# neale/safelife-k2

Hardware: AMD Instinct MI355X
Metric: env-steps/sec (whole node) on 64×64 boards, batch 65536; bit-exact vs CPU ref (higher is better)
Workload: dtype u16; 1 GPU; 64x64 proc-gen prune-still, PPO wrapper chain; envs_per_gpu=65536, burnin_steps=400, global_batch=65536, parallelism=dp1 (env shards), obs=none, rng=philox, board_mode=auto, read_board=False

## Files before the change

include/safelife_hip.h:

```cpp
#ifndef SAFELIFE_HIP_H
#define SAFELIFE_HIP_H

#include <stdint.h>

#ifdef __cplusplus
extern "C" {
#endif

#define SL_OK 0
#define SL_EINVAL (-1)
#define SL_EHIP (-2)
#define SL_ETOOBIG (-3)

#define SL_RNG_STREAM 0
#define SL_RNG_PHILOX 1

#define SL_KERNEL_AUTO 0
#define SL_KERNEL_GENERIC 1
#define SL_KERNEL_FAST 2
#define SL_KERNEL_BANDS 3
#define SL_KERNEL_MID 4

#define SL_FAMILY_GENERIC 0
#define SL_FAMILY_SMALL_SEG4 1
// ... 139 lines not shown
    int32_t *possible;
    int32_t *side_effect;
    float *spawn_prob;
    double *min_performance;
    int32_t *prior_x;
    int32_t *prior_y;
    int32_t *prior_len;
    int32_t *prior_head;
    int32_t *exit_count;
    int16_t *exit_y, *exit_x;
    int32_t *level_index;
    int32_t *episodes;
    int32_t *num_steps;
    int32_t *spawn_flags;
    int32_t *start_roll;
    uint32_t *planes;
    int32_t *planes_ok;
    uint32_t *elig_planes;
    uint32_t *board_planes;
    uint32_t board_zero;
    int32_t planes_live;
    uint32_t agent_planes;
    uint32_t goals_gray;
} sl_env_state;

enum sl_planes_ok_bits {
    SL_POK_GOALS_MIRROR = 2,
    SL_POK_GOALS_FIXED = 4,
    SL_POK_ELIG = 8,
    SL_POK_GOALS_SIX = 16,
    SL_POK_GOALS_LEVEL = 32,
    SL_POK_BOARD_PLANES = 64,
    SL_POK_BOARD_FULL = 128,
    SL_POK_BOARD_LO12 = 256,
    SL_POK_GOALS = SL_POK_GOALS_MIRROR | SL_POK_GOALS_FIXED | SL_POK_GOALS_SIX |
                   SL_POK_GOALS_LEVEL,
    SL_POK_BOARD = SL_POK_BOARD_PLANES | SL_POK_BOARD_FULL | SL_POK_BOARD_LO12
};

typedef struct sl_level_pool {
    int32_t K, H, W;
    const uint16_t *board;
    const uint16_t *goals;
    const int32_t *agent_x, *agent_y, *orientation;
    const float *spawn_prob;
    const double *min_performance;
// ... 74 lines not shown
#define SL_PLAN_K64_BITS64 1
#define SL_PLAN_K64_PLANES 2
#define SL_PLAN_K64_GRAY 3
#define SL_PLAN_K64_W6 4
#define SL_PLAN_K64_S6 5
#define SL_PLAN_K64_CHAN 6
#define SL_PLAN_KEEP_RUNTIME 0
#define SL_PLAN_KEEP_C3 1
#define SL_PLAN_KEEP_ALL 2

typedef struct sl_step_plan {
    int32_t empty;
    int32_t family;
    int32_t replay;
    int32_t stream_phase;
    int32_t plane_mode;
    int32_t demote_first;
    int32_t obs;
    int32_t resets;
    int32_t capture;
    int32_t kernel64;
    int32_t keep;
    int32_t view_kind;
} sl_step_plan;

int sl_env_step_plan(const sl_env_state *st, const sl_level_pool *pool, const sl_env_cfg *cfg,
                     const uint8_t *info_flags, sl_step_plan *out);

int sl_env_board_sync(sl_env_state *st, void *stream);

int sl_env_reset(sl_env_state *st, const sl_level_pool *pool, const uint8_t *mask,
                 const sl_env_cfg *cfg, void *stream);

int sl_env_obs(const sl_env_state *st, int vh, int vw, int remove_white_goals,
               int obs_mode, const int32_t *channels, int nch, void *out,
               void *stream);

int sl_env_action(sl_env_state *st, const int32_t *actions, int can_toggle_powers,
                  int can_toggle_colors, int64_t *act, void *stream);
int sl_env_advance(sl_env_state *st, const sl_env_cfg *cfg, void *stream);
int sl_env_rescore(sl_env_state *st, int32_t *points, void *stream);
int sl_env_exit_colors(sl_env_state *st, int mode, void *stream);


int sl_sample_actions(const void *probs, int probs_f64, int64_t B, int A, int64_t ld,
                      int rng_mode, const double *uniforms, uint64_t seed, uint32_t env0,
// ... 12 lines not shown
```

safelife-k2_amd/csrc/sl_bits.hip:

```cpp
#include "sl_bits_geo.h"
#include "sl_env_step.h"

using namespace sl;
using namespace sl::fast;
using namespace sl::bits;

namespace {

constexpr int kMinWaves = 4;
constexpr int kMinWavesObs = 3;

constexpr int N = 64;

typedef __attribute__((address_space(3))) u32 lds_u32;

__device__ __forceinline__ void dma_board(const uint16_t *__restrict__ src, lds_u32 *buf,
                                          int lane) {
    const char *s = reinterpret_cast<const char *>(src);
#pragma unroll
    for (int k = 0; k < 8; k++) {
        const int q = k * 64 + lane, row = q >> 3, pos = q & 7;
        const int c = (pos - ((row >> 5) << 2)) & 7;
        __builtin_amdgcn_global_load_lds((const void *)(s + row * 128 + c * 16),
                                         (__attribute__((address_space(3))) void *)(buf + k * 256),
// ... 631 lines not shown
    }
    if (fx.fuse_reset && reset && lane == 0) queue_reset(fx.scratch, st.B, a.step, b);
}

template <int OBS, int MODE>
__global__ void __launch_bounds__(64, (OBS || MODE == SPAWN_STREAM) ? kMinWavesObs : kMinWaves)
k_env_step_bits64(StepKArgs ka) {
    const int64_t b = blockIdx.x;
    const int lane = threadIdx.x;
    __shared__ __attribute__((aligned(16))) u32 stage[N * N / 2];
    __shared__ __attribute__((aligned(16))) uint16_t vmask[OBS >= 2 ? sl::obs::kFusedChanCells : 2];
    __shared__ uint8_t rowlist[OBS ? 64 : 1];
    lds_u32 *buf = (lds_u32 *)&stage[0];
    Pre pre;
    issue_pre(ka.st, ka.actions, b, lane, pre);
    dma_board(ka.st.board + b * (int64_t)(N * N), buf, lane);
    step_env<OBS, MODE>(ka.st, ka.a, ka.fx, b, lane, buf, vmask, rowlist, ka.actions, ka.ctp, ka.ctc,
                        ka.reward_out, ka.done_out, ka.flags_out, ka.ep_len_out, ka.ep_rew_out,
                        pre);
}


constexpr u32 kKeepAll = 0xFFFFu, kKeepC3 = 0x877Fu, kAgentC3 = 0x0062u;
template <u32 K16>
struct PlaneSlots {
    static constexpr bool kFixed = K16 == kKeepC3;
    u32 keep;
    u32 store;
    __device__ __forceinline__ u32 keep32() const { return K16 ? K16 * 0x10001u : keep; }
    __device__ __forceinline__ u32 store32() const {
        return kFixed ? (K16 & ~kAgentC3) * 0x10001u : store;
    }
    __device__ __forceinline__ bool kept(int q) const { return (keep32() >> q) & 1u; }
    __device__ __forceinline__ bool stored(int q) const { return (store32() >> q) & 1u; }
    __device__ __forceinline__ u32 agent16() const {
        return kFixed ? kAgentC3 : (keep32() & ~store32()) & 0xFFFFu;
    }
    __device__ __forceinline__ int pos(int q) const {
        if (kFixed) return __builtin_popcount(store32() & ((1u << q) - 1u));
        u32 k = store;
        asm volatile("" : "+s"(k));
        return __builtin_popcount(k & ((1u << q) - 1u));
    }
    __device__ __forceinline__ int stored16() const { return __builtin_popcount(store32() & 0xFFFFu); }
    static __device__ __forceinline__ PlaneSlots of(u32 zero, u32 agent) {
        const u32 k = ~zero & 0xFFFFu;
        return PlaneSlots{k * 0x10001u, (k & ~agent) * 0x10001u};
    }
};
__device__ __forceinline__ void agent_words(int ay, int ax, int lane, u32 aw[2]) {
    const u32 bit = lane == 2 * (ax >> 1) + (ay >> 5) ? 1u << (ay & 31) : 0u;
    aw[0] = (ax & 1) ? 0u : bit;
    aw[1] = (ax & 1) ? bit : 0u;
}
constexpr int kMinWavesPlanes = 5;
constexpr int planes_min_waves(u32 k16, int obs) {
    return (obs == 0 && k16 == kKeepC3) ? kMinWavesPlanes : kMinWaves;
}

template <u32 K16>
__device__ __forceinline__ void dma_planes(const u32 *__restrict__ bp, PlaneSlots<K16> ps,
                                           lds_u32 *buf, int lane) {
    const int groups = (2 * ps.stored16() + 3) >> 2;
    const char *s = reinterpret_cast<const char *>(bp);
#pragma unroll
    for (int g = 0; g < 8; g++)
        if (g < groups)
            __builtin_amdgcn_global_load_lds((const void *)(s + g * 1024 + lane * 16),
                                             (__attribute__((address_space(3))) void *)(buf + g * 256),
                                             16, 0, 2);
}

__device__ __forceinline__ int near_cell_index(int k, int y0, int x0) {
    const int dy = k < 5 ? 0 : (k == 5 ? -1 : k == 6 ? 1 : k == 7 ? -2 : 2);
    const int dx = k >= 5 || k == 0 ? 0 : (k == 1 ? -1 : k == 2 ? 1 : k == 3 ? -2 : 2);
    return ((y0 + dy) & 63) * 64 + ((x0 + dx) & 63);
}
struct NearCells {
    int y0, x0;
    u32 v;
    __device__ __forceinline__ uint32_t operator()(int i) const {
        const int dy = (((i >> 6) - y0 + 32) & 63) - 32, dx = (((i & 63) - x0 + 32) & 63) - 32;
        const int k = dy == 0 ? (dx == 0 ? 0 : dx == -1 ? 1 : dx == 1 ? 2 : dx == -2 ? 3 : 4)
                              : (dy == -1 ? 5 : dy == 1 ? 6 : dy == -2 ? 7 : 8);
        return (u32)__builtin_amdgcn_readlane((int)v, __builtin_amdgcn_readfirstlane(k));
    }
};
template <u32 K16>
__device__ __forceinline__ u32 lds_plane_cell(const lds_u32 *buf, PlaneSlots<K16> ps, int i) {
    const int y = i >> 6, x = i & 63;
    const lds_u32 *q = buf + 2 * (x >> 1) + (y >> 5);
    const u32 r = (u32)(y & 31);
    const int w = 16 * (x & 1);
    u32 v = 0;
#pragma unroll
    for (int p = 0; p < 16; p++) {
        const int pw = ps.pos(p) + (w ? ps.stored16() : 0);
        if (ps.stored(p)) v |= ((q[pw * 64] >> r) & 1u) << p;
    }
    return v;
}

template <u32 K16, int OBS>
__global__ void __launch_bounds__(64, planes_min_waves(K16, OBS))
k_env_step_bits64_planes(StepKArgs ka) {
    __shared__ __attribute__((aligned(16))) u32 stage[N * N / 2];
    uint16_t *const vm = nullptr;
    constexpr bool GRAY = false, W6 = false, SPLIT_EPI = false;
#include "sl_planes64_step.inc"
}

template <u32 K16, int OBS>
__global__ void __launch_bounds__(64, planes_min_waves(K16, OBS))
k_env_planes64_gray(StepKArgs ka) {
    static_assert(OBS <= 1, "channel views load the three colour planes");
    __shared__ __attribute__((aligned(16))) u32 stage[N * N / 2];
    uint16_t *const vm = nullptr;
    constexpr bool GRAY = true, W6 = false, SPLIT_EPI = false;
#include "sl_planes64_step.inc"
}

constexpr int kMinWavesW6 = 6;
constexpr int kStageDwW6 = 1536;
template <u32 K16>
__global__ void __launch_bounds__(64, kMinWavesW6)
k_env_planes64_w6(StepKArgs ka) {
    __shared__ __attribute__((aligned(16))) u32 stage[kStageDwW6];
    uint16_t *const vm = nullptr;
    constexpr int OBS = 0;
    constexpr bool GRAY = true, W6 = true, SPLIT_EPI = false;
#include "sl_planes64_step.inc"
}

template <u32 K16>
__global__ void __launch_bounds__(64, kMinWavesW6)
k_env_planes64_s6(StepKArgs ka) {
    __shared__ __attribute__((aligned(16))) u32 stage[kStageDwW6];
    uint16_t *const vm = nullptr;
    constexpr int OBS = 0;
    constexpr bool GRAY = true, W6 = true, SPLIT_EPI = true;
#include "sl_planes64_step.inc"
}

constexpr int kTailThreads = 256;
__global__ void __launch_bounds__(kTailThreads)
k_env_epilogue_reset64(sl_env_state st, StepArgs a, sl_level_pool pool, ResetArgs ra,
                       int64_t *scratch, double *reward_out, uint8_t *done_out,
                       uint8_t *flags_out, int32_t *ep_len_out, int32_t *ep_rew_out) {
    const int64_t b = (int64_t)blockIdx.x * kTailThreads + threadIdx.x;
    const int lane = threadIdx.x & 63;
    if (b == 0) scratch[8 * st.B + 2 + ((a.step + 1) & 1)] = 0;
    bool reset = false;
    if (b < st.B) {
        const Handover h = get_handover(handover_of(scratch, st.B), b);
        const HandFields f{{st, b, a.bonus_table}, h.go, h.ax, h.ay};
        reset = epilogue_core(st, a, b, f, h.act_reward, h.points, h.score, h.possible, h.side,
                              reward_out, done_out, flags_out, ep_len_out, ep_rew_out);
    }
    __shared__ uint64_t finished[kTailThreads / 64];
    const int wave = __builtin_amdgcn_readfirstlane((int)(threadIdx.x >> 6));
    const uint64_t mine = __ballot(reset);
    if (lane == 0) finished[wave] = mine;
    __builtin_amdgcn_fence(__ATOMIC_RELEASE, "workgroup");
// ... 1 lines not shown
    const int64_t b0 = (int64_t)blockIdx.x * kTailThreads;
    int i = 0;
#pragma unroll 1
    for (int q = 0; q < kTailThreads / 64; q++) {
        const uint64_t f = finished[q];
        uint64_t todo = ((uint64_t)(u32)__builtin_amdgcn_readfirstlane((int)(f >> 32)) << 32) |
                        (u32)__builtin_amdgcn_readfirstlane((int)f);
        while (todo) {
            const int k = __builtin_ctzll(todo);
            todo &= todo - 1;
            if ((i++ & (kTailThreads / 64 - 1)) == wave) wave_reset(st, pool, ra, b0 + 64 * q + k, lane);
        }
    }
}

template <u32 K16, int ESZ>
__global__ void __launch_bounds__(64, kMinWaves)
k_env_planes64_chan(StepKArgs ka) {
    constexpr int OBS = ESZ == 1 ? 3 : (ESZ == 4 ? 4 : 2);
    __shared__ __attribute__((aligned(16))) u32 stage[N * N / 2];
    __shared__ __attribute__((aligned(16))) uint16_t vmask[sl::obs::kFusedChanCells];
    uint16_t *const vm = vmask;
    constexpr bool GRAY = false, W6 = false, SPLIT_EPI = false;
#include "sl_planes64_step.inc"
}

__global__ void __launch_bounds__(64) k_board_sync64(sl_env_state st, int demote) {
    const int64_t b = blockIdx.x;
    const int lane = threadIdx.x;
    const int pok = __builtin_amdgcn_readfirstlane(st.planes_ok[b]);
    if (!(pok & SL_POK_BOARD_PLANES)) return;
    if (!(pok & SL_POK_BOARD_FULL)) {
        const PlaneSlots<0> ps = PlaneSlots<0>::of(st.board_zero, st.agent_planes);
        const u32 *bp = st.planes + b * 4096 + lane;
        u32 P[32];
#pragma unroll
        for (int q = 0; q < 32; q++) P[q] = ps.stored(q) ? bp[ps.pos(q) * 64] : 0u;
        u32 aw[2];
        agent_words(__builtin_amdgcn_readfirstlane(st.agent_y[b]),
                    __builtin_amdgcn_readfirstlane(st.agent_x[b]), lane, aw);
#pragma unroll
        for (int q = 0; q < 32; q++)
            if ((ps.agent16() >> (q & 15)) & 1u) P[q] = aw[q >> 4];
        transpose32(P);
        u32 *gb = reinterpret_cast<u32 *>(st.board + b * (int64_t)(N * N)) + (lane & 1) * 1024 +
                  (lane >> 1);
#pragma unroll
        for (int y = 0; y < 32; y++) gb[y * 32] = P[y];
    }
    if (lane == 0)
        st.planes_ok[b] = demote ? pok & ~(SL_POK_BOARD_PLANES | SL_POK_BOARD_FULL)
                                 : pok | SL_POK_BOARD_FULL;
}

__global__ void __launch_bounds__(64)
k_stream_prologue64(StepKArgs ka) {
    const sl_env_state &st = ka.st;
    const int64_t b = blockIdx.x;
    const int lane = threadIdx.x;
    const int64_t off = b * (int64_t)(N * N);
    const int lane_off = (lane & 1) * 1024 + (lane >> 1);
    const u32 V = load_record(st, ka.actions, b, lane);
    const Scratch w = scratch_of(ka.fx.scratch, st.B);
    const int spf = rec(V, R_SPF) | (ka.ctp ? 1 : 0);
    SpawnCtx sc{0u, 0u, 0ull, 0.0};
    u32 P[32], ch[2];
// ... 93 lines not shown

void launch_planes64(int keep, int obs, unsigned grid, const StepKArgs &ka, hipStream_t s) {
    switch (keep) {
    case SL_PLAN_KEEP_C3: launch_planes64_k<kKeepC3>(obs, grid, ka, s); break;
    case SL_PLAN_KEEP_ALL: launch_planes64_k<kKeepAll>(obs, grid, ka, s); break;
    default: launch_planes64_k<0>(obs, grid, ka, s); break;
    }
}

StepKArgs kargs_of(const StepCall &c) {
    return StepKArgs{*c.st, c.a, c.fx, c.actions, c.ctp, c.ctc, c.reward, c.done, c.flags,
                     c.ep_len, c.ep_rew};
}

int counts64(const StepCall &c) {
    const sl_env_state &st = *c.st;
    const int rc = launch_env_action(st, c.actions, c.ctp, c.ctc,
                                     scratch_of(c.fx.scratch, st.B).act, c.s);
    if (rc) return rc;
    hipLaunchKernelGGL(k_stream_prologue64, dim3((unsigned)st.B), dim3(64), 0, c.s, kargs_of(c));
    return hipGetLastError() == hipSuccess ? SL_OK : SL_EHIP;
}

int step64(const StepCall &c) {
    const StepPlan &p = c.plan;
    const unsigned grid = (unsigned)c.st->B;
    const StepKArgs ka = kargs_of(c);
    hipStream_t s = c.s;
    switch (p.kernel64) {
    case SL_PLAN_K64_BITS64:
        if (p.replay) launch_bits64<SPAWN_STREAM>(p.view_kind, grid, ka, s);
        else launch_bits64<SPAWN_PHILOX>(p.view_kind, grid, ka, s);
        break;
    case SL_PLAN_K64_PLANES: launch_planes64(p.keep, p.view_kind, grid, ka, s); break;
    case SL_PLAN_K64_CHAN: launch_planes64_chan(p.keep, obs_esz(p.view_kind), grid, ka, s); break;
    case SL_PLAN_K64_GRAY:
        if (p.view_kind)
            hipLaunchKernelGGL((k_env_planes64_gray<kKeepC3, 1>), dim3(grid), dim3(64), 0, s, ka);
        else
            hipLaunchKernelGGL((k_env_planes64_gray<kKeepC3, 0>), dim3(grid), dim3(64), 0, s, ka);
        break;
    case SL_PLAN_K64_S6:
        hipLaunchKernelGGL((k_env_planes64_s6<kKeepC3>), dim3(grid), dim3(64), 0, s, ka);
        break;
    case SL_PLAN_K64_W6:
        hipLaunchKernelGGL((k_env_planes64_w6<kKeepC3>), dim3(grid), dim3(64), 0, s, ka);
        break;
    default: return SL_EINVAL;
    }
    return hipGetLastError() == hipSuccess ? SL_OK : SL_EHIP;
}
// ... 44 lines not shown
```

safelife-k2_amd/csrc/sl_env_step.hip:

```cpp
#include "sl_env_step.h"

using namespace sl;

namespace {

constexpr bool kAutoTakesMid = true;

int view_kind_of(int obs_mode) {
    switch (obs_mode) {
    case SL_OBS_PACKED: return 1;
    case SL_OBS_CHANNELS_U8: return 3;
    case SL_OBS_CHANNELS_F32: return 4;
    default: return 2;
    }
}

}

extern "C" int sl_env_step_family(int H, int W, int kernel) {
    if (H < 1 || W < 1) return SL_EINVAL;
    if (kernel != SL_KERNEL_AUTO && kernel != SL_KERNEL_GENERIC && kernel != SL_KERNEL_FAST)
        return SL_EINVAL;
    if (kernel != SL_KERNEL_GENERIC) {
        if (H == 64 && W == 64) return SL_FAMILY_BITS64;
// ... 61 lines not shown
                         p.oa.vh <= kViewMaxRows128 && p.oa.vw <= 128;
    const bool fuse64 =
        fast && cfg.obs_out &&
        ((p.oa.mode == SL_OBS_PACKED && p.oa.vh * p.oa.vw <= obs::kObsMaxCells) ||
         (p.oa.mode != SL_OBS_PACKED && p.oa.vh <= 64 && p.oa.vw <= 64 &&
          p.oa.vh * p.oa.vw + 2 <= obs::kFusedChanCells && (((uintptr_t)cfg.obs_out) & 15) == 0));
    p.obs = !cfg.obs_out ? SL_PLAN_OBS_NONE
            : fuse128    ? SL_PLAN_OBS_FUSED128
            : fuse64     ? SL_PLAN_OBS_FUSED64
                         : SL_PLAN_OBS_SEPARATE;
    const bool views_ok = p.obs != SL_PLAN_OBS_SEPARATE;
    if (fast128 && planes128)
        p.plane_mode = planes_can && views_ok && (!replay || st.elig_planes);
    else if (fast && planes64)
        p.plane_mode = planes_can && views_ok && !replay;
    p.demote_first = (planes128 || planes64) && !p.plane_mode;
    p.view_kind = (p.obs == SL_PLAN_OBS_FUSED64 || p.obs == SL_PLAN_OBS_FUSED128)
                      ? view_kind_of(p.oa.mode) : 0;

    if (fast && !p.plane_mode) {
        p.kernel64 = SL_PLAN_K64_BITS64;
    } else if (fast) {
        p.keep = planes64_keep(st);
        const bool gray = p.keep == SL_PLAN_KEEP_C3 && st.goals_gray;
        if (p.view_kind >= 2) p.kernel64 = SL_PLAN_K64_CHAN;
        else if (!gray) p.kernel64 = SL_PLAN_K64_PLANES;
        else if (p.view_kind || cfg.planes64_waves == 5) p.kernel64 = SL_PLAN_K64_GRAY;
        else if (cfg.planes64_waves != SL_PLANES64_W6_UNSPLIT && cfg.auto_reset &&
                 (reinterpret_cast<uintptr_t>(cfg.scratch) & 15) == 0)
            p.kernel64 = SL_PLAN_K64_S6;
        else p.kernel64 = SL_PLAN_K64_W6;
    }

    p.resets = !cfg.auto_reset                    ? SL_PLAN_RESETS_NONE
               : small                            ? (p.cap ? SL_PLAN_RESETS_SCAN : SL_PLAN_RESETS_IN_KERNEL)
               : p.kernel64 == SL_PLAN_K64_S6     ? SL_PLAN_RESETS_SPLIT_TAIL64
               : fast                             ? SL_PLAN_RESETS_LIST64
               : fast128                          ? SL_PLAN_RESETS_LIST128
                                                  : SL_PLAN_RESETS_SCAN;
    *out = p;
    return SL_OK;
}

extern "C" int sl_env_step_plan(const sl_env_state *st, const sl_level_pool *pool,
                                const sl_env_cfg *cfg, const uint8_t *info_flags,
                                sl_step_plan *out) {
// ... 118 lines not shown
```

safelife-k2_amd/csrc/sl_planes64_step.inc:

```
    const sl_env_state &st = ka.st;
    const StepArgs &a = ka.a;
    const FastExtra &fx = ka.fx;
    const int64_t b = blockIdx.x;
    const int lane = threadIdx.x;
    lds_u32 *buf = (lds_u32 *)&stage[0];
    const PlaneSlots<K16> ps = PlaneSlots<K16>::of(st.board_zero, st.agent_planes);
    constexpr int kStageDw = (int)(sizeof(stage) / sizeof(u32));
    static_assert(!W6 || (PlaneSlots<K16>::kFixed && OBS == 0), "W6: fixed planes, no views");
    static_assert(!W6 || 2 * __builtin_popcount(K16 & ~kAgentC3 & 0xFFFFu) * 64 <= kStageDw,
                  "the stored plane words fit the buffer");
    static_assert(pool_rows_dwords(K16 ? K16 : 0xFFFFu, W6) <= kStageDw,
                  "the pool's start-plane rows fit the buffer");
    static_assert(kStageDw >= (W6 ? N * N / 4 : N * N / 2), "a board, or half of one (W6)");
    Pre pre;
    const bool gray_blank = GRAY && (!OBS || fx.obs_rw != 0);
    if (!GRAY) issue_pre(st, ka.actions, b, lane, pre);
    else if (gray_blank) issue_pre<0>(st, ka.actions, b, lane, pre);
    else issue_pre<1>(st, ka.actions, b, lane, pre);
    dma_planes(st.planes + b * 4096, ps, buf, lane);
    const int64_t off = b * (int64_t)(N * N);
    const int lane_off = (lane & 1) * 1024 + (lane >> 1);
    u32 *gg = reinterpret_cast<u32 *>(st.goals + off) + lane_off;
    u32 *mg = st.planes + b * 4096 + 2048 + lane;
    u32 *bp = st.planes + b * 4096 + lane;
    const u32 V = pre.V;
    const int pok_all = rec(V, R_POK);
    const bool pin = (pok_all & SL_POK_BOARD_PLANES) != 0;
    u32 gcol[3][2];
#pragma unroll
    for (int k = 0; k < 3; k++) {
        gcol[k][0] = pre.g[k][0];
        gcol[k][1] = pre.g[k][1];
    }
// ... 11 lines not shown
    if (fx.pool.K > 0 && fx.pool.board_planes && st.start_roll) roll = rec(V, R_ROLL);
    wait_vm();
    if (!pin) {
        if (!W6) {
            dma_board(st.board + off, buf, lane);
            wait_vm();
        }
        u32 R[32];
        if (W6) board_pairs_halves(st.board + off, buf, lane, R);
        else read_pairs(buf, lane, R);
        transpose32(R);
#pragma unroll
        for (int q = 0; q < 32; q++)
            if (ps.stored(q)) buf[ps.pos(q) * 64 + lane] = R[q];
        __builtin_amdgcn_fence(__ATOMIC_SEQ_CST, "wavefront");
        __builtin_amdgcn_wave_barrier();
    }
    RecEnv env{st, b, rec(V, R_GO), rec(V, R_AX), rec(V, R_AY), rec(V, R_SCORE),
               rec(V, R_BASE), rec(V, R_POSS), rec_f64(V, R_MP)};
    int act_reward = 0;
    int eidx[4];
    u32 eval[4];
    const int ay0 = rec(V, R_AY), ax0 = rec(V, R_AX);
    const u32 near = lane < 9 ? lds_plane_cell(buf, ps, near_cell_index(lane, ay0, ax0)) |
                                    (lane == 0 ? ps.agent16() : 0u)
                              : 0u;
    OverlayT<NearCells> ov;
    ov.src = NearCells{ay0, ax0, near};
    ov.n = 0;
#pragma unroll
    for (int k = 0; k < 4; k++) {
        ov.idx[k] = 0;
        ov.val[k] = 0;
    }
    if (lane == 0) act_reward = act_core(env, rec(V, R_ACT), N, N, ka.ctp, ka.ctc, ov);
    int ne = ov.n;
#pragma unroll
    for (int k = 0; k < 4; k++) {
        eidx[k] = ov.idx[k];
        eval[k] = ov.val[k];
    }
    act_reward = __builtin_amdgcn_readfirstlane(act_reward);
    ne = __builtin_amdgcn_readfirstlane(ne);
#pragma unroll
    for (int k = 0; k < 4; k++) {
        eidx[k] = __builtin_amdgcn_readfirstlane(eidx[k]);
        eval[k] = (u32)__builtin_amdgcn_readfirstlane((int)eval[k]);
        if (K16) eval[k] &= K16;
        eval[k] &= ~ps.agent16();
    }
    const RecFields fl = rec_fields(a, V, __builtin_amdgcn_readfirstlane(env.go),
                                    __builtin_amdgcn_readfirstlane(env.ax),
                                    __builtin_amdgcn_readfirstlane(env.ay));

    u32 PB[32];
#pragma unroll
    for (int q = 0; q < 32; q++) PB[q] = ps.stored(q) ? buf[ps.pos(q) * 64 + lane] : 0u;
    wait_lgkm();
    constexpr u32 KEEP = K16 ? K16 : 0xFFFFu;
    if (roll < 0) {
        if (!W6) dma_board(st.start_board + off, buf, lane);
    } else pool_dma<KEEP, W6>(fx.pool, rec(V, R_LI), buf, lane);
    (void)mux_edits(PB, ne, eidx, eval, lane);
    {
        u32 aw[2];
        agent_words(fl.ay, fl.ax, lane, aw);
#pragma unroll
        for (int q = 0; q < 32; q++)
            if ((ps.agent16() >> (q & 15)) & 1u) PB[q] = aw[q >> 4];
    }
    u32 cb[2], held[2];
    rule_planes(PB, cb, Geo64<SPAWN_PHILOX>{lane, ssrc, 0, 0}, sc, 0u, held);
    const uint64_t held_lanes = __ballot((held[0] | held[1]) != 0u);
#pragma unroll
    for (int w = 0; w < 2; w++) asm volatile("" : "+v"(PL(PB, 3, w)));
    __builtin_amdgcn_sched_barrier(0);

    u32 PS[32];
    wait_vm();
    if (roll >= 0) {
        if (!W6) pool_planes_lds<KEEP>(buf, roll >> 16, roll & 0xFFFF, lane, PS);
    } else {
        if (W6) board_pairs_halves(st.start_board + off, buf, lane, PS);
        else read_pairs(buf, lane, PS);
        transpose32(PS);
#pragma unroll
        for (int q = 0; q < 32; q++)
            if (!((KEEP >> (q & 15)) & 1u)) PS[q] = 0u;
    }
    int pts, scr, pos, side;
    const u32 gblack[3][2] = {{0u, 0u}, {0u, 0u}, {0u, 0u}};
    if (W6 && roll >= 0) {
// ... 95 lines not shown
```

safelife-k2_amd/safelife_amd/_lib.py:

```python
import ctypes
import os
import subprocess

_HERE = os.path.dirname(os.path.abspath(__file__))
_DEFAULT_LIB = os.path.join(_HERE, "_native", "libsafelife_hip.so")
LIB_PATH = os.environ.get("SAFELIFE_HIP_LIB") or _DEFAULT_LIB
CSRC = os.path.join(os.path.dirname(_HERE), "csrc")

SL_OK, SL_EINVAL, SL_EHIP, SL_ETOOBIG = 0, -1, -2, -3
SL_RNG_STREAM, SL_RNG_PHILOX = 0, 1
SL_KERNEL_AUTO, SL_KERNEL_GENERIC, SL_KERNEL_FAST = 0, 1, 2
SL_KERNEL_BANDS = 3
SL_KERNEL_MID = 4
(SL_FAMILY_GENERIC, SL_FAMILY_SMALL_SEG4, SL_FAMILY_SMALL, SL_FAMILY_MID, SL_FAMILY_BITS64,
 SL_FAMILY_BITS128) = range(6)
FAMILY_NAMES = {SL_FAMILY_GENERIC: "generic", SL_FAMILY_SMALL_SEG4: "small-seg4",
                SL_FAMILY_SMALL: "small", SL_FAMILY_MID: "mid", SL_FAMILY_BITS64: "bits64",
                SL_FAMILY_BITS128: "bits128"}
SL_PLAN_OBS_NONE, SL_PLAN_OBS_FUSED64, SL_PLAN_OBS_FUSED128, SL_PLAN_OBS_SEPARATE = range(4)
(SL_PLAN_RESETS_NONE, SL_PLAN_RESETS_IN_KERNEL, SL_PLAN_RESETS_LIST64,
 SL_PLAN_RESETS_SPLIT_TAIL64, SL_PLAN_RESETS_LIST128, SL_PLAN_RESETS_SCAN) = range(6)
(SL_PLAN_K64_NONE, SL_PLAN_K64_BITS64, SL_PLAN_K64_PLANES, SL_PLAN_K64_GRAY, SL_PLAN_K64_W6,
 SL_PLAN_K64_S6, SL_PLAN_K64_CHAN) = range(7)
SL_PLAN_KEEP_RUNTIME, SL_PLAN_KEEP_C3, SL_PLAN_KEEP_ALL = range(3)
# ... 15 lines not shown
           SL_ETOOBIG: "board too large for this kernel"}

vp = ctypes.c_void_p
i32 = ctypes.c_int32
i64 = ctypes.c_int64
u32 = ctypes.c_uint32
u64 = ctypes.c_uint64
f32 = ctypes.c_float
f64 = ctypes.c_double


class EnvState(ctypes.Structure):
    _fields_ = [("B", i64), ("H", i32), ("W", i32),
                ("board", vp), ("goals", vp), ("start_board", vp),
                ("agent_x", vp), ("agent_y", vp), ("orientation", vp),
                ("game_over", vp), ("episode_length", vp), ("episode_reward", vp),
                ("old_points", vp), ("baseline", vp), ("score", vp), ("possible", vp),
                ("side_effect", vp), ("spawn_prob", vp), ("min_performance", vp),
                ("prior_x", vp), ("prior_y", vp), ("prior_len", vp), ("prior_head", vp),
                ("exit_count", vp), ("exit_y", vp), ("exit_x", vp),
                ("level_index", vp), ("episodes", vp), ("num_steps", vp),
                ("spawn_flags", vp), ("start_roll", vp), ("planes", vp), ("planes_ok", vp),
                ("elig_planes", vp), ("board_planes", vp), ("board_zero", u32),
                ("planes_live", i32), ("agent_planes", u32), ("goals_gray", u32)]


class LevelPool(ctypes.Structure):
    _fields_ = [("K", i32), ("H", i32), ("W", i32),
                ("board", vp), ("goals", vp), ("agent_x", vp), ("agent_y", vp),
                ("orientation", vp), ("spawn_prob", vp), ("min_performance", vp),
                ("board_planes", vp), ("goal_planes", vp)]


class EnvCfg(ctypes.Structure):
    _fields_ = [("time_limit", i32), ("auto_reset", i32),
                ("can_toggle_powers", i32), ("can_toggle_colors", i32),
                ("penalty_coef", f64), ("wrapper_min_performance", f64),
                ("bonus_table", vp), ("bonus_len", i32), ("bonus_period", i32),
                ("rng_mode", i32), ("seed", u64), ("step", u32), ("env0", u32),
                ("draws", vp), ("n_draws", i64), ("stream_pos", vp), ("scratch", vp),
                ("level_mode", i32), ("n_total_envs", i32), ("augment_roll", i32),
                ("ev_begin", vp), ("ev_end", vp), ("kernel", i32),
                ("obs_out", vp), ("obs_mode", i32), ("obs_vh", i32), ("obs_vw", i32),
                ("obs_remove_white", i32), ("obs_nch", i32), ("obs_channels", i32 * 16),
                ("capture", vp), ("stream_phase", i32), ("stream_base", vp), ("mt", vp),
                ("board_mode", i32), ("planes64_waves", i32)]


class StepPlan(ctypes.Structure):
    _fields_ = [(n, i32) for n in ("empty", "family", "replay", "stream_phase", "plane_mode",
                                   "demote_first", "obs", "resets", "capture", "kernel64",
                                   "keep", "view_kind")]


class MT19937(ctypes.Structure):
    _fields_ = [("n_chains", i32), ("rounds", i32), ("ring_draws", i64), ("ring", vp),
                ("chains", vp), ("prefix", vp), ("polys", vp), ("ctl", vp),
                ("ahead_stream", vp), ("ev_fill", vp), ("ev_ahead", vp),
                ("ahead_pending", i32), ("bit_ring", i32), ("bits_thr", f64)]


class Capture(ctypes.Structure):
    _fields_ = [("n", i32), ("env", vp), ("board", vp), ("goals", vp), ("orientation", vp),
                ("flags", vp), ("reset_board", vp), ("reset_goals", vp),
                ("reset_orientation", vp),
                ("start_board", vp), ("score", vp), ("possible", vp), ("baseline", vp),
                ("num_steps", vp), ("spawn_prob", vp), ("min_performance", vp),
                ("episode_length", vp), ("episode_reward", vp), ("level_index", vp)]


_lib = None


class HipUnavailable(RuntimeError):
    pass
# ... 139 lines not shown
```

safelife-k2_amd/safelife_amd/vec_env.py:

```python
import ctypes
import math

import numpy as np

from . import _lib
from .levels import LevelPool
from .spaces import Box, env_spaces

ACTION_NAMES = ("NULL", "MOVE UP", "MOVE RIGHT", "MOVE DOWN", "MOVE LEFT",
                "TOGGLE UP", "TOGGLE RIGHT", "TOGGLE DOWN", "TOGGLE LEFT")


class GlobalCounter:

    def __init__(self):
        self.episodes_started = 0
        self.episodes_completed = 0
        self.num_steps = 0


def _sched(val, counter):
    return val(counter.num_steps) if callable(val) else val


# ... 13 lines not shown
    board = np.asarray(board, dtype=np.uint16)
    K = board.shape[0]
    if K == 0:
        return 0
    cand = AGENT_PLANE_BITS & ~(0x00E1 if can_toggle_powers else 0)
    at = board[np.arange(K), np.asarray(agent_y), np.asarray(agent_x)]
    if not (at & 0x0010).all():
        return 0
    mask = 0
    for k in range(16):
        bit = 1 << k
        if not cand & bit:
            continue
        n = ((board & bit) != 0).reshape(K, -1).sum(1)
        if (n == 1).all() and ((at & bit) != 0).all():
            mask |= bit
    return mask


def goals_gray(goals):
    g = np.asarray(goals, dtype=np.uint16)
    r, gr, b = (g >> 9) & 1, (g >> 10) & 1, (g >> 11) & 1
    return int(bool(((r == gr) & (r == b)).all()))


def start_board_hi_bits(start_board):
    import torch
    return ((start_board.view(torch.int16) & 0x7000) != 0).flatten(1).any(1)


class SafeLifeVecEnv:
    action_names = ACTION_NAMES

    def __init__(self, levels, num_envs, device=None, *, time_limit=1000,
                 view_shape=(15, 15), output_channels=tuple(range(15)),
                 remove_white_goals=True, movement_bonus=0.1, movement_bonus_power=0.01,
                 movement_bonus_period=4, penalty_coef=0.0, min_performance=0.01,
                 auto_reset=True, rng="philox", seed=0, spawn_stream=None,
                 level_order="sequential", augment_roll=False, env0=0, n_total_envs=None,
                 can_toggle_powers=False, can_toggle_colors=False, obs_dtype="uint16",
                 compute_obs=True, global_counter=None, kernel="auto", stream_exchange=None,
                 stream_ring="auto", board_mode="auto", planes64_waves=6):
        import torch
        self.torch = torch
        self.device = _lib.require_device(device)
        self.pool = levels if isinstance(levels, LevelPool) else LevelPool.from_levels(levels)
# ... 80 lines not shown
            "exit_y": z(B, _lib.SL_MAX_EXITS, dt=torch.int16),
            "exit_x": z(B, _lib.SL_MAX_EXITS, dt=torch.int16),
            "level_index": z(B), "episodes": z(B), "num_steps": z(B), "spawn_flags": z(B),
            "start_roll": z(B) - 1,
        }
        s = _lib.EnvState()
        s.B, s.H, s.W = B, H, W
        s.board, s.goals, s.start_board = (self._board.data_ptr(), self.goals.data_ptr(),
                                           self.start_board.data_ptr())
        for k, t in self.st_t.items():
            setattr(s, k, t.data_ptr())
        self.planes_ok = z(B)
        if (H, W) in ((64, 64), (128, 128)):
            self.planes = z(B, H // 32, 32, 64)
            s.planes = self.planes.data_ptr()
            s.planes_ok = self.planes_ok.data_ptr()
        self.board_planes = None
        if (H, W) == (64, 64):
            self.board_planes = self.planes
            s.board_planes = self.planes.data_ptr()
            s.board_zero = self._zero_planes(self._pool_bits(self.pool))
            s.agent_planes = self._agent_planes(self.pool)
            s.goals_gray = goals_gray(self.pool.goals)
        if (H, W) == (128, 128):
            self.board_planes = z(B, H // 32, 32, 64)
            s.board_planes = self.board_planes.data_ptr()
            s.board_zero = self._zero_planes(self._pool_bits(self.pool))
        if (H, W) == (128, 128) and self.rng == "stream":
            self.elig_planes = z(B, 1024)
            s.elig_planes = self.elig_planes.data_ptr()
        self._state = s
        self.actions_dev = z(B)
        self.reward = z(B, dt=torch.float64)
        self.done = z(B, dt=torch.uint8)
        self.flags = z(B, dt=torch.uint8)
        self.ep_len = z(B)
        self.ep_rew = z(B)
        self.scratch = z(8 * B + 16, dt=torch.int64)
        self.stream_pos = z(1, dt=torch.int64)
        vh, vw = self.view_shape
        if self.output_channels is None:
            self.obs_mode = _lib.SL_OBS_PACKED
            self.obs = z(B, vh, vw, dt=torch.uint16)
        else:
            nch = len(self.output_channels)
            modes = {"uint16": (_lib.SL_OBS_CHANNELS, torch.uint16),
# ... 18 lines not shown
    def _allow_board_bits(self, bits):
        s = self._state
        if not s.board_zero:
            return
        new = s.board_zero & self._zero_planes(bits)
        if new != s.board_zero:
            self.sync_board()
            self._pok_clear(_lib.SL_POK_BOARD)
            s.board_zero = new
            s.planes_live = 0

    def _agent_planes(self, pool):
        return agent_planes(pool.board, pool.agent_x, pool.agent_y, self.can_toggle_powers)

    def _narrow_agent_planes(self, keep=0):
        s = self._state
        new = s.agent_planes & keep
        if new != s.agent_planes:
            self.sync_board()
            self._pok_clear(_lib.SL_POK_BOARD)
            s.agent_planes = new
            s.planes_live = 0

    def _narrow_goals_gray(self, keep=0):
        self._state.goals_gray &= int(keep)

    def _admit_pool_boards(self, pool):
        self._allow_board_bits(self._pool_bits(pool))
        self._narrow_agent_planes(self._agent_planes(pool))
        self._narrow_goals_gray(goals_gray(pool.goals))
        self._may_spawn = self._may_spawn or pool.has_spawners()

    def _device_board_bits(self, boards):
        v = boards.view(self.torch.int16)
        return sum(1 << k for k in range(16) if bool(((v >> k) & 1).any().item()))

    def _pok_clear(self, bits, e=None):
        (self.planes_ok if e is None else self.planes_ok[e]).bitwise_and_(~bits)

    def _pok_goals_written(self, e=None):
        self.sync_board()
        self._pok_clear(_lib.SL_POK_GOALS, e)

    def _pok_board_written(self, e=None):
        self._pok_clear(_lib.SL_POK_ELIG | _lib.SL_POK_BOARD, e)

    def _pok_state_replaced(self, e=None):
        (self.planes_ok if e is None else self.planes_ok[e]).zero_()

    def _pok_stepping_switched(self, e=None):
        self._pok_clear(_lib.SL_POK_ELIG, e)

    def _cells(self, cells):
        torch = self.torch
        if not isinstance(cells, torch.Tensor):
            cells = torch.from_numpy(np.ascontiguousarray(cells, dtype=np.uint16))
        if tuple(cells.shape) != (self.H, self.W):
            raise ValueError("board must be %dx%d" % (self.H, self.W))
        return cells.to(device=self.device, dtype=torch.uint16)

    def write_board(self, e, cells):
        v = self._cells(cells)
        self._allow_board_bits(self._device_board_bits(v))
        self._narrow_agent_planes()
        self._synced_board()[e].copy_(v)
        self.st_t["spawn_flags"][e].bitwise_or_(1)
        self._may_spawn = True
        self._pok_board_written(e)

    def write_goals(self, e, cells):
        self._narrow_goals_gray()
        self.goals[e].copy_(self._cells(cells))
        self.st_t["spawn_flags"][e].bitwise_or_(2)
        self._may_spawn = True
        self._pok_goals_written(e)

    def set_pool(self, levels, pool_dev=None):
        pool = levels if isinstance(levels, LevelPool) else LevelPool.from_levels(levels)
        if (pool.H, pool.W) != (self.H, self.W):
            raise ValueError("pool boards are %dx%d, the env's %dx%d"
                             % (pool.H, pool.W, self.H, self.W))
        if pool.K < 1:
            raise ValueError("empty level pool")
        self._admit_pool_boards(pool)
        self.pool = pool
        self._pool_dev = pool_dev if pool_dev is not None else pool.to_device(self.device)
        self._check_ring_threshold(pool.spawn_prob)
# ... 330 lines not shown

    def _out(self, t, default):
        if t is None:
            return default
        if (t.shape != default.shape or t.dtype != default.dtype or t.device != self.device
                or not t.is_contiguous()):
            raise ValueError("output must be a contiguous %s %s tensor on %s"
                             % (tuple(default.shape), default.dtype, self.device))
        return t

    def step_wait(self):
        info = {"times_up": (self.flags & 1) != 0, "game_over": (self.flags & 2) != 0,
                "reset": (self.flags & 4) != 0, "episode_length": self.ep_len,
                "episode_reward": self.ep_rew}
        return (self.obs if self.compute_obs else None), self.reward, self.done.bool(), info

    def state_slice(self, i0, n=1):
        if not (0 <= i0 and n >= 0 and i0 + n <= self.B):
            raise IndexError("env slice [%d, %d) outside [0, %d)" % (i0, i0 + n, self.B))
        full, s = self._state, _lib.EnvState()
        s.B, s.H, s.W = n, self.H, self.W
        for name, _ in _lib.EnvState._fields_[3:]:
            base = getattr(full, name)
            if name in ("board_zero", "planes_live", "agent_planes",
                        "goals_gray"):
                setattr(s, name, base)
                continue
            if not base:
                setattr(s, name, None)
                continue
            t = self._state_tensor(name)
            setattr(s, name, base + i0 * (t.stride(0) * t.element_size()))
        return s

    def _state_tensor(self, name):
        if name == "board":
            return self._board
        if name in ("goals", "start_board", "planes", "planes_ok", "elig_planes", "board_planes"):
            return getattr(self, name)
        return self.st_t[name]

    @property
    def board(self):
        self._board_read_at = self._step_index
        return self._synced_board()

    def _synced_board(self):
        self.sync_board()
# ... 9 lines not shown
    @property
    def state(self):
        return self.st_t

    def stream_error(self):
        return bool(self.scratch[8 * self.B].item()
                    & (_lib.SL_STREAM_ERR_RANGE | _lib.SL_STREAM_ERR_THRESHOLD))

    def set_state(self, board, goals, start_board, **scalars):
        torch = self.torch
        for dst, src in ((self._board, board), (self.goals, goals), (self.start_board, start_board)):
            dst.copy_(torch.as_tensor(np.ascontiguousarray(src, dtype=np.uint16)).to(self.device))
        for k, v in scalars.items():
            t = self.st_t[k]
            t.copy_(torch.as_tensor(np.asarray(v)).to(device=self.device, dtype=t.dtype))
        self._invalidate_caches()

    def _invalidate_caches(self):
        self.st_t["start_roll"].fill_(-1)
        if self._state.board_zero:
            self._state.board_zero &= self._zero_planes(self._device_board_bits(self._board)
                                                        | self._device_board_bits(self.start_board))
        self._state.agent_planes = 0
        self._narrow_goals_gray()
        hi = start_board_hi_bits(self.start_board) & ((self.H, self.W) == (128, 128))
        self.st_t["spawn_flags"].copy_(3 | 4 * hi.to(self.st_t["spawn_flags"].dtype))
        self._may_spawn = True
        self._pok_state_replaced()
        self.scratch[8 * self.B + 2:8 * self.B + 4].zero_()
        self._last_step = None
        self._check_ring_threshold()
        self._synced = (int(self.st_t["episodes"].sum().item()),
                        int(self.st_t["episodes"].sum().item())
                        - int(self._running_mask().sum().item()) - self._abandoned)

    def state_dict(self):
        d = {"board": self._synced_board().clone(), "goals": self.goals.clone(),
             "start_board": self.start_board.clone(), "step_index": self._step_index,
             "stream_pos": self.stream_pos.clone()}
        pos = getattr(self.stream_exchange, "pos", None)
        if pos is not None:
            d["exchange_pos"] = pos.clone()
        d.update({k: v.clone() for k, v in self.st_t.items()})
        d["agent_planes"] = self.torch.tensor(int(self._state.agent_planes),
                                              dtype=self.torch.int32)
        d["goals_gray"] = self.torch.tensor(int(self._state.goals_gray),
                                            dtype=self.torch.int32)
        return d

    def load_state_dict(self, d):
        li = d["level_index"]
        if int(li.min().item()) < 0 or int(li.max().item()) >= self.pool.K:
            import warnings
            warnings.warn("state_dict level_index outside the current pool of %d levels"
                          " (informational only)" % self.pool.K)
        self._board.copy_(d["board"])
        self.goals.copy_(d["goals"])
        self.start_board.copy_(d["start_board"])
        for k, v in self.st_t.items():
            v.copy_(d[k])
        self._step_index = int(d["step_index"])
        self.stream_pos.copy_(d["stream_pos"])
        pos = getattr(self.stream_exchange, "pos", None)
        if pos is not None and "exchange_pos" in d:
            pos.copy_(d["exchange_pos"])
        if self.mt is not None:
            self.mt.seek(int((pos if pos is not None else self.stream_pos).item()))
        ap = self._state.agent_planes & int(d.get("agent_planes", 0))
        gg = self._state.goals_gray & int(d.get("goals_gray", 0))
        self._invalidate_caches()
        self._state.agent_planes = ap
        self._state.goals_gray = gg
```

Baseline: 618.3 million env-steps/s.

## Derive bit-15 and exit planes instead of storing them in planes layout

Adds a derived_planes mask. When the pool shows that bit 15 always mirrors bit 2 (powers cannot be toggled) and that exit cells are few and recorded in per-env exit lists, those two bit-planes are no longer stored or DMA'd. Instead they are rebuilt in registers from plane 2 and the exit coordinates. For the C3 keep set this shrinks the stored planes from 16 words to 12, which is three DMA groups instead of four, and adds a specialised kernel family that drops them. The cost is extra per-step reconstruction work, an exit loop in the cell lookups, and host-side bookkeeping that must narrow the mask whenever boards change.

```diff
diff --git a/include/safelife_hip.h b/include/safelife_hip.h
--- a/include/safelife_hip.h
+++ b/include/safelife_hip.h
@@ -185,6 +185,7 @@
     int32_t planes_live;
     uint32_t agent_planes;
     uint32_t goals_gray;
+    uint32_t derived_planes;
 } sl_env_state;
 
 enum sl_planes_ok_bits {
@@ -305,6 +306,8 @@
     int32_t kernel64;
     int32_t keep;
     int32_t view_kind;
+    int32_t stored;
+    int32_t derived;
 } sl_step_plan;
 
 int sl_env_step_plan(const sl_env_state *st, const sl_level_pool *pool, const sl_env_cfg *cfg,
diff --git a/safelife-k2_amd/csrc/sl_bits.hip b/safelife-k2_amd/csrc/sl_bits.hip
--- a/safelife-k2_amd/csrc/sl_bits.hip
+++ b/safelife-k2_amd/csrc/sl_bits.hip
@@ -677,32 +677,59 @@
 
 
 constexpr u32 kKeepAll = 0xFFFFu, kKeepC3 = 0x877Fu, kAgentC3 = 0x0062u;
-template <u32 K16>
+constexpr u32 kDerivable = 0x8100u;
+__host__ __device__ constexpr u32 derived_eff(u32 derived) {
+    return (derived & kDerivable) == kDerivable ? kDerivable : 0u;
+}
+template <u32 K16, int DM = -1>
 struct PlaneSlots {
     static constexpr bool kFixed = K16 == kKeepC3;
     u32 keep;
     u32 store;
+    u32 drv_;
+    __device__ __forceinline__ u32 drv16() const { return DM >= 0 ? (u32)DM : drv_; }
     __device__ __forceinline__ u32 keep32() const { return K16 ? K16 * 0x10001u : keep; }
     __device__ __forceinline__ u32 store32() const {
         return kFixed ? (K16 & ~kAgentC3) * 0x10001u : store;
     }
+    static constexpr bool late(int q) { return (kDerivable >> (q & 15)) & 1u; }
     __device__ __forceinline__ bool kept(int q) const { return (keep32() >> q) & 1u; }
-    __device__ __forceinline__ bool stored(int q) const { return (store32() >> q) & 1u; }
+    __device__ __forceinline__ bool laid(int q) const { return (store32() >> q) & 1u; }
+    __device__ __forceinline__ bool stored(int q) const {
+        return laid(q) && !(late(q) && ((drv16() >> (q & 15)) & 1u));
+    }
+    __device__ __forceinline__ u32 stored32() const { return store32() & ~(drv16() * 0x10001u); }
     __device__ __forceinline__ u32 agent16() const {
         return kFixed ? kAgentC3 : (keep32() & ~store32()) & 0xFFFFu;
     }
     __device__ __forceinline__ int pos(int q) const {
-        if (kFixed) return __builtin_popcount(store32() & ((1u << q) - 1u));
-        u32 k = store;
+        const u32 below = (1u << q) - 1u;
+        if (kFixed && DM >= 0) return __builtin_popcount(stored32() & below);
+        u32 k = stored32();
         asm volatile("" : "+s"(k));
-        return __builtin_popcount(k & ((1u << q) - 1u));
-    }
-    __device__ __forceinline__ int stored16() const { return __builtin_popcount(store32() & 0xFFFFu); }
-    static __device__ __forceinline__ PlaneSlots of(u32 zero, u32 agent) {
+        return __builtin_popcount(k & below);
+    }
+    __device__ __forceinline__ int stored16() const {
+        return __builtin_popcount(stored32() & 0xFFFFu);
+    }
+    static __device__ __forceinline__ PlaneSlots of(u32 zero, u32 agent, u32 derived) {
         const u32 k = ~zero & 0xFFFFu;
-        return PlaneSlots{k * 0x10001u, (k & ~agent) * 0x10001u};
+        const u32 s = kFixed ? (K16 & ~kAgentC3) : ((K16 ? K16 : k) & ~agent);
+        return PlaneSlots{k * 0x10001u, (k & ~agent) * 0x10001u, derived_eff(derived) & s};
     }
 };
+__device__ __forceinline__ void exit_words(u32 V, int lane, u32 ew[2]) {
+    const RecFields fl{V, 0, 0, 0, 0.0};
+    const int n = min(fl.exit_count(), SL_MAX_EXITS);
+    ew[0] = ew[1] = 0u;
+#pragma unroll 1
+    for (int e = 0; e < n; e++) {
+        const int y = fl.exit_y(e), x = fl.exit_x(e);
+        const u32 bit = lane == 2 * (x >> 1) + (y >> 5) ? 1u << (y & 31) : 0u;
+        if (x & 1) ew[1] |= bit;
+        else ew[0] |= bit;
+    }
+}
 __device__ __forceinline__ void agent_words(int ay, int ax, int lane, u32 aw[2]) {
     const u32 bit = lane == 2 * (ax >> 1) + (ay >> 5) ? 1u << (ay & 31) : 0u;
     aw[0] = (ax & 1) ? 0u : bit;
@@ -713,8 +740,8 @@
     return (obs == 0 && k16 == kKeepC3) ? kMinWavesPlanes : kMinWaves;
 }
 
-template <u32 K16>
-__device__ __forceinline__ void dma_planes(const u32 *__restrict__ bp, PlaneSlots<K16> ps,
+template <u32 K16, int DM>
+__device__ __forceinline__ void dma_planes(const u32 *__restrict__ bp, PlaneSlots<K16, DM> ps,
                                            lds_u32 *buf, int lane) {
     const int groups = (2 * ps.stored16() + 3) >> 2;
     const char *s = reinterpret_cast<const char *>(bp);
@@ -741,8 +768,9 @@
         return (u32)__builtin_amdgcn_readlane((int)v, __builtin_amdgcn_readfirstlane(k));
     }
 };
-template <u32 K16>
-__device__ __forceinline__ u32 lds_plane_cell(const lds_u32 *buf, PlaneSlots<K16> ps, int i) {
+template <u32 K16, int DM>
+__device__ __forceinline__ u32 lds_plane_cell(const lds_u32 *buf, PlaneSlots<K16, DM> ps, u32 V,
+                                              int i) {
     const int y = i >> 6, x = i & 63;
     const lds_u32 *q = buf + 2 * (x >> 1) + (y >> 5);
     const u32 r = (u32)(y & 31);
@@ -753,15 +781,25 @@
         const int pw = ps.pos(p) + (w ? ps.stored16() : 0);
         if (ps.stored(p)) v |= ((q[pw * 64] >> r) & 1u) << p;
     }
+    if (ps.drv16() & 0x8000u) v |= (v & 4u) << 13;
+    if (ps.drv16() & 0x0100u) {
+        const RecFields fl{V, 0, 0, 0, 0.0};
+        const int n = min(fl.exit_count(), SL_MAX_EXITS);
+#pragma unroll 1
+        for (int e = 0; e < n; e++)
+            if (i == fl.exit_y(e) * 64 + fl.exit_x(e)) v |= 0x0100u;
+    }
     return v;
 }
 
+constexpr int planes_dm(u32 k16) { return k16 == kKeepC3 ? (int)kDerivable : -1; }
 template <u32 K16, int OBS>
 __global__ void __launch_bounds__(64, planes_min_waves(K16, OBS))
 k_env_step_bits64_planes(StepKArgs ka) {
     __shared__ __attribute__((aligned(16))) u32 stage[N * N / 2];
     uint16_t *const vm = nullptr;
     constexpr bool GRAY = false, W6 = false, SPLIT_EPI = false;
+    constexpr int DM = planes_dm(K16);
 #include "sl_planes64_step.inc"
 }
 
@@ -772,6 +810,7 @@
     __shared__ __attribute__((aligned(16))) u32 stage[N * N / 2];
     uint16_t *const vm = nullptr;
     constexpr bool GRAY = true, W6 = false, SPLIT_EPI = false;
+    constexpr int DM = planes_dm(K16);
 #include "sl_planes64_step.inc"
 }
 
@@ -784,6 +823,7 @@
     uint16_t *const vm = nullptr;
     constexpr int OBS = 0;
     constexpr bool GRAY = true, W6 = true, SPLIT_EPI = false;
+    constexpr int DM = planes_dm(K16);
 #include "sl_planes64_step.inc"
 }
 
@@ -794,6 +834,7 @@
     uint16_t *const vm = nullptr;
     constexpr int OBS = 0;
     constexpr bool GRAY = true, W6 = true, SPLIT_EPI = true;
+    constexpr int DM = planes_dm(K16);
 #include "sl_planes64_step.inc"
 }
 
@@ -841,6 +882,22 @@
     __shared__ __attribute__((aligned(16))) uint16_t vmask[sl::obs::kFusedChanCells];
     uint16_t *const vm = vmask;
     constexpr bool GRAY = false, W6 = false, SPLIT_EPI = false;
+    constexpr int DM = planes_dm(K16);
+#include "sl_planes64_step.inc"
+}
+
+constexpr int stored16_min_waves(int kind, int obs) {
+    return kind == 2 || kind == 3 ? kMinWavesW6 : (kind == 4 ? kMinWaves : planes_min_waves(kKeepC3, obs));
+}
+template <int KIND, int OBS>
+__global__ void __launch_bounds__(64, stored16_min_waves(KIND, OBS))
+k_env_p64_stored16(StepKArgs ka) {
+    constexpr u32 K16 = kKeepC3;
+    constexpr int DM = 0;
+    constexpr bool GRAY = KIND >= 1 && KIND <= 3, W6 = KIND == 2 || KIND == 3, SPLIT_EPI = KIND == 3;
+    __shared__ __attribute__((aligned(16))) u32 stage[W6 ? kStageDwW6 : N * N / 2];
+    __shared__ __attribute__((aligned(16))) uint16_t vmask[OBS >= 2 ? sl::obs::kFusedChanCells : 2];
+    uint16_t *const vm = OBS >= 2 ? vmask : nullptr;
 #include "sl_planes64_step.inc"
 }
 
@@ -850,7 +907,8 @@
     const int pok = __builtin_amdgcn_readfirstlane(st.planes_ok[b]);
     if (!(pok & SL_POK_BOARD_PLANES)) return;
     if (!(pok & SL_POK_BOARD_FULL)) {
-        const PlaneSlots<0> ps = PlaneSlots<0>::of(st.board_zero, st.agent_planes);
+        const PlaneSlots<0> ps = PlaneSlots<0>::of(st.board_zero, st.agent_planes,
+                                                   st.derived_planes);
         const u32 *bp = st.planes + b * 4096 + lane;
         u32 P[32];
 #pragma unroll
@@ -861,6 +919,21 @@
 #pragma unroll
         for (int q = 0; q < 32; q++)
             if ((ps.agent16() >> (q & 15)) & 1u) P[q] = aw[q >> 4];
+        if (ps.drv16() & 0x8000u) {
+            PL(P, 15, 0) = PL(P, 2, 0);
+            PL(P, 15, 1) = PL(P, 2, 1);
+        }
+        if (ps.drv16() & 0x0100u) {
+            const int n = min(__builtin_amdgcn_readfirstlane(st.exit_count[b]), SL_MAX_EXITS);
+            PL(P, 8, 0) = PL(P, 8, 1) = 0u;
+            for (int e = 0; e < n; e++) {
+                const int y = __builtin_amdgcn_readfirstlane(st.exit_y[b * SL_MAX_EXITS + e]);
+                const int x = __builtin_amdgcn_readfirstlane(st.exit_x[b * SL_MAX_EXITS + e]);
+                const u32 bit = lane == 2 * (x >> 1) + (y >> 5) ? 1u << (y & 31) : 0u;
+                if (x & 1) PL(P, 8, 1) |= bit;
+                else PL(P, 8, 0) |= bit;
+            }
+        }
         transpose32(P);
         u32 *gb = reinterpret_cast<u32 *>(st.board + b * (int64_t)(N * N)) + (lane & 1) * 1024 +
                   (lane >> 1);
@@ -1000,11 +1073,37 @@
     return hipGetLastError() == hipSuccess ? SL_OK : SL_EHIP;
 }
 
+#define SL_STORED16(KIND, OBS) \
+    hipLaunchKernelGGL((k_env_p64_stored16<KIND, OBS>), dim3(grid), dim3(64), 0, s, ka)
+bool launch_stored16(const StepPlan &p, unsigned grid, const StepKArgs &ka, hipStream_t s) {
+    switch (p.kernel64) {
+    case SL_PLAN_K64_PLANES:
+        if (p.view_kind) SL_STORED16(0, 1);
+        else SL_STORED16(0, 0);
+        return true;
+    case SL_PLAN_K64_GRAY:
+        if (p.view_kind) SL_STORED16(1, 1);
+        else SL_STORED16(1, 0);
+        return true;
+    case SL_PLAN_K64_W6: SL_STORED16(2, 0); return true;
+    case SL_PLAN_K64_S6: SL_STORED16(3, 0); return true;
+    case SL_PLAN_K64_CHAN:
+        if (p.view_kind == 3) SL_STORED16(4, 3);
+        else if (p.view_kind == 4) SL_STORED16(4, 4);
+        else SL_STORED16(4, 2);
+        return true;
+    default: return false;
+    }
+}
+#undef SL_STORED16
+
 int step64(const StepCall &c) {
     const StepPlan &p = c.plan;
     const unsigned grid = (unsigned)c.st->B;
     const StepKArgs ka = kargs_of(c);
     hipStream_t s = c.s;
+    if (p.keep == SL_PLAN_KEEP_C3 && p.derived == 0 && launch_stored16(p, grid, ka, s))
+        return hipGetLastError() == hipSuccess ? SL_OK : SL_EHIP;
     switch (p.kernel64) {
     case SL_PLAN_K64_BITS64:
         if (p.replay) launch_bits64<SPAWN_STREAM>(p.view_kind, grid, ka, s);
diff --git a/safelife-k2_amd/csrc/sl_env_step.hip b/safelife-k2_amd/csrc/sl_env_step.hip
--- a/safelife-k2_amd/csrc/sl_env_step.hip
+++ b/safelife-k2_amd/csrc/sl_env_step.hip
@@ -107,6 +107,9 @@
         p.kernel64 = SL_PLAN_K64_BITS64;
     } else if (fast) {
         p.keep = planes64_keep(st);
+        const uint32_t laid = ~st.board_zero & ~st.agent_planes & 0xFFFFu;
+        p.derived = (int32_t)(((st.derived_planes & 0x8100u) == 0x8100u ? 0x8100u : 0u) & laid);
+        p.stored = (int32_t)(laid & ~(uint32_t)p.derived);
         const bool gray = p.keep == SL_PLAN_KEEP_C3 && st.goals_gray;
         if (p.view_kind >= 2) p.kernel64 = SL_PLAN_K64_CHAN;
         else if (!gray) p.kernel64 = SL_PLAN_K64_PLANES;
diff --git a/safelife-k2_amd/csrc/sl_planes64_step.inc b/safelife-k2_amd/csrc/sl_planes64_step.inc
--- a/safelife-k2_amd/csrc/sl_planes64_step.inc
+++ b/safelife-k2_amd/csrc/sl_planes64_step.inc
@@ -4,11 +4,14 @@
     const int64_t b = blockIdx.x;
     const int lane = threadIdx.x;
     lds_u32 *buf = (lds_u32 *)&stage[0];
-    const PlaneSlots<K16> ps = PlaneSlots<K16>::of(st.board_zero, st.agent_planes);
+    const PlaneSlots<K16, DM> ps = PlaneSlots<K16, DM>::of(st.board_zero, st.agent_planes,
+                                                           st.derived_planes);
     constexpr int kStageDw = (int)(sizeof(stage) / sizeof(u32));
-    static_assert(!W6 || (PlaneSlots<K16>::kFixed && OBS == 0), "W6: fixed planes, no views");
-    static_assert(!W6 || 2 * __builtin_popcount(K16 & ~kAgentC3 & 0xFFFFu) * 64 <= kStageDw,
-                  "the stored plane words fit the buffer");
+    static_assert(!W6 || (PlaneSlots<K16, DM>::kFixed && OBS == 0), "W6: fixed planes, no views");
+    constexpr int kStoredWords =
+        2 * __builtin_popcount(K16 & ~kAgentC3 & ~(u32)(DM > 0 ? DM : 0) & 0xFFFFu);
+    static_assert(K16 != kKeepC3 || kStoredWords == (DM ? 12 : 16), "three DMA groups, or four");
+    static_assert(!W6 || kStoredWords * 64 <= kStageDw, "the stored plane words fit the buffer");
     static_assert(pool_rows_dwords(K16 ? K16 : 0xFFFFu, W6) <= kStageDw,
                   "the pool's start-plane rows fit the buffer");
     static_assert(kStageDw >= (W6 ? N * N / 4 : N * N / 2), "a board, or half of one (W6)");
@@ -66,7 +69,7 @@
     int eidx[4];
     u32 eval[4];
     const int ay0 = rec(V, R_AY), ax0 = rec(V, R_AX);
-    const u32 near = lane < 9 ? lds_plane_cell(buf, ps, near_cell_index(lane, ay0, ax0)) |
+    const u32 near = lane < 9 ? lds_plane_cell(buf, ps, V, near_cell_index(lane, ay0, ax0)) |
                                     (lane == 0 ? ps.agent16() : 0u)
                               : 0u;
     OverlayT<NearCells> ov;
@@ -112,6 +115,16 @@
 #pragma unroll
         for (int q = 0; q < 32; q++)
             if ((ps.agent16() >> (q & 15)) & 1u) PB[q] = aw[q >> 4];
+    }
+    if (ps.drv16() & 0x8000u) {
+#pragma unroll
+        for (int w = 0; w < 2; w++) PL(PB, 15, w) = PL(PB, 2, w);
+    }
+    if (ps.drv16() & 0x0100u) {
+        u32 ew[2];
+        exit_words(V, lane, ew);
+#pragma unroll
+        for (int w = 0; w < 2; w++) PL(PB, 8, w) = ew[w];
     }
     u32 cb[2], held[2];
     rule_planes(PB, cb, Geo64<SPAWN_PHILOX>{lane, ssrc, 0, 0}, sc, 0u, held);
diff --git a/safelife-k2_amd/safelife_amd/_lib.py b/safelife-k2_amd/safelife_amd/_lib.py
--- a/safelife-k2_amd/safelife_amd/_lib.py
+++ b/safelife-k2_amd/safelife_amd/_lib.py
@@ -61,7 +61,8 @@
                 ("level_index", vp), ("episodes", vp), ("num_steps", vp),
                 ("spawn_flags", vp), ("start_roll", vp), ("planes", vp), ("planes_ok", vp),
                 ("elig_planes", vp), ("board_planes", vp), ("board_zero", u32),
-                ("planes_live", i32), ("agent_planes", u32), ("goals_gray", u32)]
+                ("planes_live", i32), ("agent_planes", u32), ("goals_gray", u32),
+                ("derived_planes", u32)]
 
 
 class LevelPool(ctypes.Structure):
@@ -89,7 +90,7 @@
 class StepPlan(ctypes.Structure):
     _fields_ = [(n, i32) for n in ("empty", "family", "replay", "stream_phase", "plane_mode",
                                    "demote_first", "obs", "resets", "capture", "kernel64",
-                                   "keep", "view_kind")]
+                                   "keep", "view_kind", "stored", "derived")]
 
 
 class MT19937(ctypes.Structure):
diff --git a/safelife-k2_amd/safelife_amd/vec_env.py b/safelife-k2_amd/safelife_amd/vec_env.py
--- a/safelife-k2_amd/safelife_amd/vec_env.py
+++ b/safelife-k2_amd/safelife_amd/vec_env.py
@@ -59,6 +59,23 @@
     g = np.asarray(goals, dtype=np.uint16)
     r, gr, b = (g >> 9) & 1, (g >> 10) & 1, (g >> 11) & 1
     return int(bool(((r == gr) & (r == b)).all()))
+
+
+DERIVABLE_PLANE_BITS = 0x8100
+
+
+def derived_planes(board, can_toggle_powers=False):
+    b = np.asarray(board, dtype=np.uint16)
+    if b.shape[0] == 0:
+        return 0
+    mask = 0
+    if not can_toggle_powers and bool((((b >> 2) & 1) == ((b >> 15) & 1)).all()):
+        mask |= 0x8000
+    ex = b[(b & 0x0100) != 0]
+    if (int(((b & 0x0100) != 0).reshape(b.shape[0], -1).sum(1).max()) <= 8
+            and bool(((ex & 0x0010) != 0).all()) and not bool((ex & 0x800C).any())):
+        mask |= 0x0100
+    return mask
 
 
 def start_board_hi_bits(start_board):
@@ -185,6 +202,7 @@
             s.board_zero = self._zero_planes(self._pool_bits(self.pool))
             s.agent_planes = self._agent_planes(self.pool)
             s.goals_gray = goals_gray(self.pool.goals)
+            s.derived_planes = self._derived_planes(self.pool)
         if (H, W) == (128, 128):
             self.board_planes = z(B, H // 32, 32, 64)
             s.board_planes = self.board_planes.data_ptr()
@@ -249,12 +267,25 @@
             s.agent_planes = new
             s.planes_live = 0
 
+    def _derived_planes(self, pool):
+        return derived_planes(pool.board, self.can_toggle_powers)
+
+    def _narrow_derived_planes(self, keep=0):
+        s = self._state
+        new = s.derived_planes & keep
+        if new != s.derived_planes:
+            self.sync_board()
+            self._pok_clear(_lib.SL_POK_BOARD)
+            s.derived_planes = new
+            s.planes_live = 0
+
     def _narrow_goals_gray(self, keep=0):
         self._state.goals_gray &= int(keep)
 
     def _admit_pool_boards(self, pool):
         self._allow_board_bits(self._pool_bits(pool))
         self._narrow_agent_planes(self._agent_planes(pool))
+        self._narrow_derived_planes(self._derived_planes(pool))
         self._narrow_goals_gray(goals_gray(pool.goals))
         self._may_spawn = self._may_spawn or pool.has_spawners()
 
@@ -290,6 +321,7 @@
         v = self._cells(cells)
         self._allow_board_bits(self._device_board_bits(v))
         self._narrow_agent_planes()
+        self._narrow_derived_planes()
         self._synced_board()[e].copy_(v)
         self.st_t["spawn_flags"][e].bitwise_or_(1)
         self._may_spawn = True
@@ -666,8 +698,8 @@
         s.B, s.H, s.W = n, self.H, self.W
         for name, _ in _lib.EnvState._fields_[3:]:
             base = getattr(full, name)
-            if name in ("board_zero", "planes_live", "agent_planes",
-                        "goals_gray"):
+            if name in ("board_zero", "planes_live", "agent_planes", "goals_gray",
+                        "derived_planes"):
                 setattr(s, name, base)
                 continue
             if not base:
@@ -723,6 +755,7 @@
             self._state.board_zero &= self._zero_planes(self._device_board_bits(self._board)
                                                         | self._device_board_bits(self.start_board))
         self._state.agent_planes = 0
+        self._state.derived_planes = 0
         self._narrow_goals_gray()
         hi = start_board_hi_bits(self.start_board) & ((self.H, self.W) == (128, 128))
         self.st_t["spawn_flags"].copy_(3 | 4 * hi.to(self.st_t["spawn_flags"].dtype))
@@ -747,6 +780,8 @@
                                               dtype=self.torch.int32)
         d["goals_gray"] = self.torch.tensor(int(self._state.goals_gray),
                                             dtype=self.torch.int32)
+        d["derived_planes"] = self.torch.tensor(int(self._state.derived_planes),
+                                                dtype=self.torch.int32)
         return d
 
     def load_state_dict(self, d):
@@ -769,6 +804,8 @@
             self.mt.seek(int((pos if pos is not None else self.stream_pos).item()))
         ap = self._state.agent_planes & int(d.get("agent_planes", 0))
         gg = self._state.goals_gray & int(d.get("goals_gray", 0))
+        dp = self._state.derived_planes & int(d.get("derived_planes", 0))
         self._invalidate_caches()
         self._state.agent_planes = ap
         self._state.goals_gray = gg
+        self._state.derived_planes = dp
```

Result: faster. 657.4 million env-steps/s (median of 6 runs) (+6.3%).
